# TuringLang/AdvancedVI.jl

Hardware: AMD Instinct MI355X
Metric: ELBO-grad-estimates/sec (higher is better)
Workload: dtype f32

## Files before the change

advancedvi.jl_amd/csrc/device_common.h:

```cpp
#pragma once
#include "mivi_internal.h"
#include "philox.h"
#include <type_traits>

namespace mivi {

template <typename T>
__device__ __forceinline__ T wave_sum(T v) {
#pragma unroll
  for (int o = 32; o > 0; o >>= 1) v += __shfl_xor(v, o, 64);
  return v;
}

__device__ __forceinline__ float wave_sum_f32(float v) {
  v += __builtin_bit_cast(float, __builtin_amdgcn_update_dpp(0, __builtin_bit_cast(int, v), 0xB1, 0xF, 0xF, true));
  v += __builtin_bit_cast(float, __builtin_amdgcn_update_dpp(0, __builtin_bit_cast(int, v), 0x4E, 0xF, 0xF, true));
  v += __builtin_bit_cast(float, __builtin_amdgcn_update_dpp(0, __builtin_bit_cast(int, v), 0x141, 0xF, 0xF, true));
  v += __builtin_bit_cast(float, __builtin_amdgcn_update_dpp(0, __builtin_bit_cast(int, v), 0x140, 0xF, 0xF, true));
  const int iv = __builtin_bit_cast(int, v);
  return __builtin_bit_cast(float, __builtin_amdgcn_readlane(iv, 0)) + __builtin_bit_cast(float, __builtin_amdgcn_readlane(iv, 16)) +
         __builtin_bit_cast(float, __builtin_amdgcn_readlane(iv, 32)) + __builtin_bit_cast(float, __builtin_amdgcn_readlane(iv, 48));
}
__device__ __forceinline__ double wave_sum_fast(float v) { return (double)wave_sum_f32(v); }
__device__ __forceinline__ double wave_sum_fast(double v) { return wave_sum(v); }

template <typename T, int NT>
__device__ __forceinline__ T block_sum(T v, T *red) {
  const int lane = threadIdx.x & 63, w = threadIdx.x >> 6;
  v = wave_sum(v);
  __syncthreads();
  if (lane == 0) red[w] = v;
  __syncthreads();
  T s = red[0];
#pragma unroll
  for (int i = 1; i < NT / 64; ++i) s += red[i];
  return s;
}

__device__ __forceinline__ void lds_barrier();
template <typename T, int NT>
__device__ __forceinline__ T block_sum_nodrain(T v, T *red) {
  const int lane = threadIdx.x & 63, w = threadIdx.x >> 6;
  v = wave_sum(v);
  lds_barrier();
  if (lane == 0) red[w] = v;
  lds_barrier();
  T s = red[0];
#pragma unroll
  for (int i = 1; i < NT / 64; ++i) s += red[i];
  return s;
}

template <int NT>
__device__ __forceinline__ double block_sum_nodrain_f32(float v, double *red) {
  const int lane = threadIdx.x & 63, w = threadIdx.x >> 6;
  const double sv = (double)wave_sum_f32(v);
  lds_barrier();
  if (lane == 0) red[w] = sv;
  lds_barrier();
  double s = red[0];
#pragma unroll
  for (int i = 1; i < NT / 64; ++i) s += red[i];
  return s;
}

template <typename T, int NT, int N>
__device__ __forceinline__ void block_sum_n(T (&v)[N], T *red) {
  const int lane = threadIdx.x & 63, w = threadIdx.x >> 6;
#pragma unroll
  for (int k = 0; k < N; ++k) v[k] = wave_sum(v[k]);
  __syncthreads();
  if (lane == 0) {
#pragma unroll
    for (int k = 0; k < N; ++k) red[k * (NT / 64) + w] = v[k];
  }
  __syncthreads();
#pragma unroll
  for (int k = 0; k < N; ++k) {
    T s = red[k * (NT / 64)];
#pragma unroll
    for (int i = 1; i < NT / 64; ++i) s += red[k * (NT / 64) + i];
    v[k] = s;
  }
}

template <int B, int E, typename F>
__device__ __forceinline__ void static_for(F &&f) {
  if constexpr (B < E) {
    f(std::integral_constant<int, B>{});
    static_for<B + 1, E>(f);
  }
}

template <typename V16>
__device__ __forceinline__ void store16_wt(void *p, const V16 &v) {
  static_assert(sizeof(V16) == 16, "16-byte vector");
  typedef unsigned u32x4_t __attribute__((ext_vector_type(4)));
  const u32x4_t r = __builtin_bit_cast(u32x4_t, v);
  asm volatile("global_store_dwordx4 %0, %1, off sc1\n\ts_nop 1" ::"v"(p), "v"(r) : "memory");
}

__device__ __forceinline__ void store4_wt(float *p, float v) {
  asm volatile("global_store_dword %0, %1, off sc1" ::"v"(p), "v"(v) : "memory");
}

#ifdef MIVI_DEV
#define MIVI_STAMP_K(dbgp, kind, slot) do { if ((dbgp) && threadIdx.x == 0 && blockIdx.x < 4096) (dbgp)[((size_t)(kind) * 4096 + blockIdx.x) * 8 + (slot)] = wall_clock64(); } while (0)
#define MIVI_KNOCKED(args, bits) ((args).knock & (bits))
#define MIVI_DEV_ONLY(...) __VA_ARGS__
#else
#define MIVI_STAMP_K(dbgp, kind, slot) do { } while (0)
#define MIVI_KNOCKED(args, bits) false
#define MIVI_DEV_ONLY(...)
#endif
#define MIVI_STAMP(dbgp, slot) MIVI_STAMP_K(dbgp, 0, slot)

__device__ __forceinline__ void lds_barrier() { asm volatile("s_waitcnt lgkmcnt(0)\n\ts_barrier" ::: "memory"); }

__device__ __forceinline__ uint64_t rng_index(const RngArgs &r) {
  return r.idx_base + (r.idx_ptr ? *r.idx_ptr : 0ull);
}

__device__ __forceinline__ double direct_entropy_coeff(int ent_kind) {
  switch (ent_kind) {
    case MIVI_ENT_CLOSED_FORM: return 1.0;
    case MIVI_ENT_CLOSED_FORM_ZERO_GRAD: return 0.0;
    case MIVI_ENT_MONTE_CARLO: return 1.0;
    case MIVI_ENT_STL: return 0.0;
    default: return -1.0;
  }
}

__device__ __forceinline__ bool ent_is_stl(int k) { return k == MIVI_ENT_STL || k == MIVI_ENT_STL_ZERO_GRAD; }
__device__ __forceinline__ bool ent_is_closed(int k) {
  return k == MIVI_ENT_CLOSED_FORM || k == MIVI_ENT_CLOSED_FORM_ZERO_GRAD;
}

template <typename T>
__device__ __forceinline__ T mf_grad_entry(double row_sum, double invM, bool scale_row, double direct, double sigma) {
#pragma clang fp contract(off)
  const double m = -row_sum * invM;
  const double e = direct / sigma;
  return (T)(scale_row ? m - e : m);
}

template <bool ATOMIC>
__device__ __forceinline__ double ld_f64(const double *p) {
  if (ATOMIC) return __hip_atomic_load(p, __ATOMIC_RELAXED, __HIP_MEMORY_SCOPE_AGENT);
  return *p;
}

template <typename T, int NT, bool ATOMIC = false>
__device__ __forceinline__ void funnel_finish(int d, const FunnelFin &f, const OutArgs &out, double &s_ell, double &sW, double &sWe) {
  const int tid = threadIdx.x;
  const T *params = (const T *)f.params;
  const double mu0 = f.row0 ? (double)__hip_atomic_load((const T *)f.row0, __ATOMIC_RELAXED, __HIP_MEMORY_SCOPE_AGENT) : (double)params[0];
  const double sg0 = f.row0 ? (double)__hip_atomic_load((const T *)f.row0 + 1, __ATOMIC_RELAXED, __HIP_MEMORY_SCOPE_AGENT) : (double)params[d];
  const uint64_t idx = rng_index(f.rng);
  const bool stl = ent_is_stl(out.ent_kind);
  const double n = (double)(d - 1), sv2 = f.sigma_v * f.sigma_v;
  for (int m = tid; m < f.M; m += NT) {
#pragma clang fp contract(off)
    T e[4];
    eps_block<T>(f.rng.seed, idx, (uint64_t)(f.rng.m_offset + m) * (uint64_t)f.d4, e);
    const double e0 = (double)e[0];
    const double e1 = (double)fma((T)sg0, e[0], (T)mu0);
    s_ell += (-e1 - e1 * e1 / (2.0 * sv2)) + (-n * e1) + e1;
    const double w = (-1.0 - e1 / sv2) + (-n) + 1.0 + (stl ? e0 / sg0 : 0.0);
    sW += w;
    sWe += w * e0;
  }
  if (f.wait_word) {
    for (int i = tid; i < f.wait_n; i += NT) {
      int budget = f.wait_budget;
      while ((int)(__hip_atomic_load(f.wait_word + i, __ATOMIC_RELAXED, __HIP_MEMORY_SCOPE_AGENT) - f.wait_val) < 0) {
        if (--budget <= 0) { if (out.status) atomicOr(out.status, 8); break; }
        __builtin_amdgcn_s_sleep(1);
      }
    }
    __syncthreads();
    asm volatile("" ::: "memory");
    if (f.mirror) {
      constexpr int UN = 8;
      for (int base = 0; base < f.mirror_n; base += UN * NT) {
        double v[UN];
#pragma unroll
        for (int u = 0; u < UN; ++u) {
          const int i = base + u * NT + tid;
          v[u] = i < f.mirror_n ? f.mirror_src[i] : 0.0;
        }
#pragma unroll
        for (int u = 0; u < UN; ++u) {
          const int i = base + u * NT + tid;
          if (i < f.mirror_n) f.mirror[i] = v[u];
        }
      }
      __syncthreads();
    }
  }
  for (int i = tid; i < f.n_part; i += NT) {
    sW += ld_f64<ATOMIC>(f.ab + i);
    sWe += ld_f64<ATOMIC>(f.ab + f.n_part + i);
  }
}

struct PartialDst {
  float *flat;
  const P2PDirectTab *tab;
  long long n, off;
  float inv_n;
};
__device__ __forceinline__ PartialDst partial_dst(const OutArgs &out) {
  PartialDst pd;
  pd.flat = (float *)out.partials;
  pd.tab = (const P2PDirectTab *)out.p2p_direct;
  pd.n = 1; pd.off = 0; pd.inv_n = 1.f;
  if (pd.tab) {
    const unsigned epoch = __hip_atomic_load(pd.tab->ctr, __ATOMIC_RELAXED, __HIP_MEMORY_SCOPE_AGENT) + 1u + (unsigned)out.p2p_gi;
    pd.n = pd.tab->n;
    pd.off = ((long long)((int)(epoch & 1u) * pd.tab->GV + out.p2p_v) * pd.tab->R + pd.tab->rank) * pd.n;
    pd.inv_n = 1.f / (float)pd.n;
  }
  return pd;
}
__device__ __forceinline__ void partial_store(const PartialDst &pd, long long idx, float v) {
  if (!pd.tab) { pd.flat[idx] = v; return; }
  int s = (int)((float)idx * pd.inv_n);
  if (s > pd.tab->R - 1) s = pd.tab->R - 1;
  while ((long long)s * pd.n > idx) --s;
  while ((long long)(s + 1) * pd.n <= idx) ++s;
  float *dst = (float *)pd.tab->stage[s] + pd.off + (idx - (long long)s * pd.n);
  __hip_atomic_store(dst, v, __ATOMIC_RELAXED, __HIP_MEMORY_SCOPE_SYSTEM);
}

template <typename T, int NT, bool ATOMIC, bool FUNNEL = false, typename DiagFn>
__device__ void finalize_value_block(int d, const ValueIn &vin, const OutArgs &out, int64_t plen, DiagFn scale_diag,
                                     double *red) {
  const int tid = threadIdx.x;
  double s_ell = 0.0, s_he = 0.0, s_ld = 0.0, bad = 0.0, sW = 0.0, sWe = 0.0;
  const bool funnel = FUNNEL && vin.fn.ab;
  if (funnel) funnel_finish<T, NT, ATOMIC>(d, vin.fn, out, s_ell, sW, sWe);
  for (int i = tid; i < vin.n_ell_part; i += NT) s_ell += ld_f64<ATOMIC>(vin.ell_part + i);
  for (int i = tid; i < vin.n_ell_part2; i += NT) s_ell += ld_f64<ATOMIC>(vin.ell_part2 + i);
  for (int i = tid; i < vin.n_ell; i += NT) s_ell += (double)((const T *)vin.ell)[i];
  for (int i = tid; i < vin.n_he_part; i += NT) s_he += ld_f64<ATOMIC>(vin.he_part + i);
  if (!out.partials_mode) {
    if (vin.ld_part) {
      for (int i = tid; i < vin.n_ld_part; i += NT) {
        s_ld += ld_f64<ATOMIC>(vin.ld_part + i);
        bad += ld_f64<ATOMIC>(vin.ld_part + vin.n_ld_part + i);
      }
    } else {
      for (int i = tid; i < d; i += NT) {
        const double c = (double)scale_diag(i);
// ... 57 lines not shown
```

advancedvi.jl_amd/csrc/fr_planes.h:

```cpp
#pragma once
#include "device_common.h"

namespace mivi {

typedef float f32x16 __attribute__((ext_vector_type(16)));
typedef float f32x4 __attribute__((ext_vector_type(4)));
typedef _Float16 f16x8 __attribute__((ext_vector_type(8)));
typedef _Float16 f16x2 __attribute__((ext_vector_type(2)));
typedef unsigned u32x4v __attribute__((ext_vector_type(4)));

constexpr int kFrag = 512;
constexpr int kSplitProducts = 3;
constexpr float kEpsScale = 2048.f;
constexpr float kEpsInv = 1.f / 2048.f;

#define FB_GLDS16(gptr, lptr, off)                                                                         \
  __builtin_amdgcn_global_load_lds((const __attribute__((address_space(1))) void *)(gptr),                 \
                                   (__attribute__((address_space(3))) void *)(lptr), 16, off, 0)

template <int N>
__device__ __forceinline__ void fb_wait_vm() {
  __builtin_amdgcn_s_waitcnt((N & 15) | (7 << 4) | (15 << 8) | ((N >> 4) << 14));
  asm volatile("" ::: "memory");
}
__device__ __forceinline__ void fb_barrier() {
  __builtin_amdgcn_s_waitcnt(0xc07f);
  asm volatile("s_barrier" ::: "memory");
}

__device__ __forceinline__ void fb_scale_of(float amax, float &s, float &inv) {
  unsigned eb = (__builtin_bit_cast(unsigned, amax) >> 23) & 0xffu;
  eb = eb < 25u ? 25u : (eb > 254u ? 254u : eb);
  s = __builtin_bit_cast(float, (267u - eb) << 23);
  inv = __builtin_bit_cast(float, (eb - 13u) << 23);
}

__device__ __forceinline__ void fb_split2(const float *x, u32x4v &uh, u32x4v &ul) {
#pragma unroll
  for (int p = 0; p < 4; ++p) {
    const float a = x[2 * p], b = x[2 * p + 1];
    const _Float16 ah = (_Float16)a, bh = (_Float16)b;
    const float ra = a - (float)ah, rb = b - (float)bh;
    const f16x2 hh = {ah, bh}, ll = {(_Float16)ra, (_Float16)rb};
    uh[p] = __builtin_bit_cast(unsigned, hh);
    ul[p] = __builtin_bit_cast(unsigned, ll);
  }
}
__device__ __forceinline__ float fb_unsplit2(const u32x4v &uh, const u32x4v &ul, int e) {
  const unsigned wh = uh[e >> 1], wl = ul[e >> 1];
  const f16x2 hh = __builtin_bit_cast(f16x2, wh), ll = __builtin_bit_cast(f16x2, wl);
  return (float)hh[e & 1] + (float)ll[e & 1];
}
__device__ __forceinline__ float fb_unsplit2_word(unsigned wh, unsigned wl, int odd) {
  const f16x2 hh = __builtin_bit_cast(f16x2, wh), ll = __builtin_bit_cast(f16x2, wl);
  return (float)hh[odd] + (float)ll[odd];
}
__device__ __forceinline__ void fb_store_frag(unsigned *dst, const float *x) {
  u32x4v uh, ul;
  fb_split2(x, uh, ul);
  store16_wt(dst, uh);
  store16_wt(dst + 256, ul);
}

constexpr int kStageW = 16 * 256;

template <int WJ>
struct FbFrags {
  u32x4v A[2][2], B[WJ][2];
};
__device__ __forceinline__ f32x16 fb_mma(const u32x4v &a, const u32x4v &b, const f32x16 &c) {
  return __builtin_amdgcn_mfma_f32_32x32x16_f16(__builtin_bit_cast(f16x8, a), __builtin_bit_cast(f16x8, b), c, 0, 0, 0);
}
template <int WJ>
__device__ __forceinline__ void fb_group(const FbFrags<WJ> &F, f32x16 (&acc)[2][WJ]) {
  constexpr int PA[3] = {1, 0, 0}, PB[3] = {0, 1, 0};
#pragma unroll
  for (int p = 0; p < 3; ++p)
#pragma unroll
    for (int i = 0; i < 2; ++i)
#pragma unroll
      for (int j = 0; j < WJ; ++j) acc[i][j] = fb_mma(F.A[i][PA[p]], F.B[j][PB[p]], acc[i][j]);
}

template <int OFF>
__device__ __forceinline__ void fb_group_read_asm(f32x16 &acc0, f32x16 &acc1, const FbFrags<1> &Fc, FbFrags<1> &Fn, unsigned ab, unsigned bb) {
  static_assert(OFF >= 0 && OFF + 3072 < 65536, "ds_read_b128 offset field");
  asm volatile(
      "v_mfma_f32_32x32x16_f16 %[c0], %[a0l], %[bh], %[c0]\n\t"
      "ds_read_b128 %[n0h], %[ab] offset:%[o0]\n\t"
      "ds_read_b128 %[n0l], %[ab] offset:%[o1]\n\t"
      "v_mfma_f32_32x32x16_f16 %[c1], %[a1l], %[bh], %[c1]\n\t"
      "ds_read_b128 %[n1h], %[ab] offset:%[o2]\n\t"
      "ds_read_b128 %[n1l], %[ab] offset:%[o3]\n\t"
      "v_mfma_f32_32x32x16_f16 %[c0], %[a0h], %[bl], %[c0]\n\t"
      "ds_read_b128 %[nbh], %[bb] offset:%[o0]\n\t"
      "v_mfma_f32_32x32x16_f16 %[c1], %[a1h], %[bl], %[c1]\n\t"
      "ds_read_b128 %[nbl], %[bb] offset:%[o1]\n\t"
      "v_mfma_f32_32x32x16_f16 %[c0], %[a0h], %[bh], %[c0]\n\t"
      "v_mfma_f32_32x32x16_f16 %[c1], %[a1h], %[bh], %[c1]\n\t"
      "s_waitcnt lgkmcnt(0)"
      : [c0] "+v"(acc0), [c1] "+v"(acc1), [n0h] "=&v"(Fn.A[0][0]), [n0l] "=&v"(Fn.A[0][1]), [n1h] "=&v"(Fn.A[1][0]), [n1l] "=&v"(Fn.A[1][1]),
        [nbh] "=&v"(Fn.B[0][0]), [nbl] "=&v"(Fn.B[0][1])
      : [a0h] "v"(Fc.A[0][0]), [a0l] "v"(Fc.A[0][1]), [a1h] "v"(Fc.A[1][0]), [a1l] "v"(Fc.A[1][1]), [bh] "v"(Fc.B[0][0]), [bl] "v"(Fc.B[0][1]),
        [ab] "v"(ab), [bb] "v"(bb), [o0] "n"(OFF), [o1] "n"(OFF + 1024), [o2] "n"(OFF + 2048), [o3] "n"(OFF + 3072)
      : "memory");
}

template <int WJ>
__device__ __forceinline__ void fb_read_frags(const unsigned *lds, int slot, int wm, int wn, int lane, FbFrags<WJ> &F) {
  const unsigned *cur = lds + slot * kStageW + 4 * lane;
#pragma unroll
  for (int i = 0; i < 2; ++i)
#pragma unroll
    for (int p = 0; p < 2; ++p) F.A[i][p] = *(const u32x4v *)(cur + ((2 * wm + i) * 2 + p) * 256);
#pragma unroll
  for (int j = 0; j < WJ; ++j)
#pragma unroll
    for (int p = 0; p < 2; ++p) F.B[j][p] = *(const u32x4v *)(cur + (8 + (WJ * wn + j) * 2 + p) * 256);
}

}
```

advancedvi.jl_amd/csrc/kernels_fullrank_batch.hip:

```cpp
#include <algorithm>
#include <cstdlib>
#include <type_traits>
#include <cstdio>
#include <vector>

#include "device_common.h"
#include "fr_elem.h"
#include "fr_planes.h"

#ifndef FB_VK
#define FB_VK 0
#endif
#ifndef FB_WJ
#define FB_WJ 1
#endif

namespace mivi {

struct FbArgs {
  int d, M, L;
  int dT, MT;
  const float *params;
  const float *t_mean, *t_istd;
  unsigned *CA;
  float *cscale;
  unsigned *epsP;
  unsigned *WV;
  float *winv;
  const float *t_prec;
  int dP;
  unsigned *PA;
  float *pscale;
  unsigned *RP;
  float *rinv;
  const float *Tinv;
  unsigned *TA;
  float *tscale;
  long long plane_stride;
  double *ell_part;
  long long ell_stride;
  double *he_part;
  long long he_stride;
  double *ld_part;
  const int4 *work;
  int n_work;
  float *grads;
  long long grad_stride;
  float *values;
  long long value_stride;
  float *grad_last, *value_last;
  int lane_last;
  int write_upper;
  int ent_kind, M_total;
  int *status;
  double ell_const;
  RngArgs rng;
  int n_riders;
  int obj;
  float *parts;
  long long part_stride;
  int knock;
  long long *dbg;
};
#ifdef MIVI_DEV
#define FB_STAMP(a, slot) do { if ((a).dbg && threadIdx.x == 0) (a).dbg[(size_t)blockIdx.x * 8 + (slot)] = (long long)wall_clock64(); } while (0)
#define FB_NOTE(a, slot, v) do { if ((a).dbg && threadIdx.x == 0) (a).dbg[(size_t)blockIdx.x * 8 + (slot)] = (long long)(v); } while (0)
#define FB_KNOCKED(a, b) ((a).knock & (b))
#else
#define FB_KNOCKED(a, b) false
#define FB_STAMP(a, slot) do { } while (0)
#define FB_NOTE(a, slot, v) do { } while (0)
#endif

template <class Ld4, class Ld>
__device__ __forceinline__ void fb_rowblock_planes(int d, int rb, int kg_lo, int kg_hi, int sub, int nsub, Ld4 ld4, Ld ld, unsigned *planes, float *scale, float *red) {
  const int tid = threadIdx.x, r4 = tid & 7, part = tid >> 3, ng = d >> 4;
  f32x4 m = {0.f, 0.f, 0.f, 0.f};
  {
    int k = 16 * kg_lo + part;
    for (; k + 448 <= 16 * kg_hi + 15; k += 512) {
      f32x4 v[8];
#pragma unroll
      for (int u = 0; u < 8; ++u) v[u] = ld4(k + 64 * u, 32 * rb + 4 * r4);
#pragma unroll
      for (int u = 0; u < 8; ++u)
#pragma unroll
        for (int c = 0; c < 4; ++c) m[c] = fmaxf(m[c], fabsf(v[u][c]));
    }
    for (; k <= 16 * kg_hi + 15; k += 64) {
      const f32x4 v = ld4(k, 32 * rb + 4 * r4);
#pragma unroll
      for (int c = 0; c < 4; ++c) m[c] = fmaxf(m[c], fabsf(v[c]));
    }
  }
#pragma unroll
  for (int c = 0; c < 4; ++c) {
    m[c] = fmaxf(m[c], __shfl_xor(m[c], 8, 64));
    m[c] = fmaxf(m[c], __shfl_xor(m[c], 16, 64));
    m[c] = fmaxf(m[c], __shfl_xor(m[c], 32, 64));
  }
  if ((tid & 63) < 8) *(f32x4 *)(red + (tid >> 6) * 32 + 4 * r4) = m;
  lds_barrier();
  if (tid < 32) {
    float mm = red[tid];
#pragma unroll
    for (int p = 1; p < 8; ++p) mm = fmaxf(mm, red[p * 32 + tid]);
    float s, inv;
    fb_scale_of(mm, s, inv);
    red[512 + tid] = s;
    if (sub == 0) {
      scale[32 * rb + tid] = s;
      scale[d + 32 * rb + tid] = inv;
    }
  }
  lds_barrier();
  const int w = tid >> 6, lane = tid & 63, l31 = lane & 31, h = lane >> 5;
  const float s = red[512 + l31];
  for (int kg = kg_lo + w + 8 * sub; kg <= kg_hi; kg += 8 * nsub) {
    float x[8];
#pragma unroll
    for (int e = 0; e < 8; ++e) x[e] = ld(16 * kg + 8 * (e >> 2) + 4 * h + (e & 3), 32 * rb + l31) * s;
    fb_store_frag(planes + ((size_t)rb * ng + kg) * kFrag + 4 * lane, x);
  }
}
__device__ __forceinline__ void fb_cplanes_block(const FbArgs &a, int rb, int sub, int nsub, float *red) {
  const int d = a.d, ng = d >> 4, dT = a.dT;
  const float *C = a.params + dT;
  const int hi = 2 * rb + 3 < ng - 1 ? 2 * rb + 3 : ng - 1;
  if (dT == d) {
    fb_rowblock_planes(d, rb, 0, hi, sub, nsub,
                       [C, d](int k, int row) { f32x4 v = *(const f32x4 *)(C + (size_t)k * d + row);
#pragma unroll
                                                for (int c = 0; c < 4; ++c) v[c] = k > row + c ? 0.f : v[c];
                                                return v; },
                       [C, d](int k, int row) { const float v = C[(size_t)k * d + row]; return k > row ? 0.f : v; }, a.CA, a.cscale, red);
    return;
  }
  fb_rowblock_planes(d, rb, 0, hi, sub, nsub,
                     [C, dT](int k, int row) { const bool in = row < dT && k < dT;
                                               f32x4 v = *(const f32x4 *)(C + (size_t)(in ? k : 0) * dT + (in ? row : 0));
#pragma unroll
                                               for (int c = 0; c < 4; ++c) v[c] = (!in || k > row + c) ? 0.f : v[c];
                                               return v; },
                     [C, dT](int k, int row) { if (row >= dT || k > row) return 0.f; return C[(size_t)k * dT + row]; }, a.CA, a.cscale, red);
}
__global__ __launch_bounds__(512) void k_fb_pplanes(FbArgs a) {
  __shared__ float red[16 * 32 + 32];
  const float *P = a.t_prec;
  const int dP = a.dP;
  fb_rowblock_planes(a.d, (int)blockIdx.x, 0, (a.d >> 4) - 1, (int)blockIdx.y, (int)gridDim.y,
                     [P, dP](int k, int row) { return *(const f32x4 *)(P + (size_t)k * dP + row); },
                     [P, dP](int k, int row) { return P[(size_t)k * dP + row]; }, a.PA, a.pscale, red);
}
__global__ __launch_bounds__(512) void k_fb_tplanes(FbArgs a) {
  __shared__ float red[16 * 32 + 32];
  const float *T = a.Tinv;
  const int d = a.d, rb = (int)blockIdx.x;
  fb_rowblock_planes(d, rb, 2 * (rb & ~3), (d >> 4) - 1, (int)blockIdx.y, (int)gridDim.y,
                     [T, d](int k, int row) { f32x4 v = *(const f32x4 *)(T + (size_t)k * d + row);
#pragma unroll
                                              for (int c = 0; c < 4; ++c) v[c] = k >= row + c ? v[c] : 0.f;
                                              return v; },
                     [T, d](int k, int row) { const float v = T[(size_t)k * d + row]; return k >= row ? v : 0.f; }, a.TA, a.tscale, red);
}

__global__ __launch_bounds__(512) void k_fb_eps(FbArgs a) {
  __shared__ double red[8];
  __shared__ float E[32 * 65];
  const int tid = threadIdx.x, eb = blockIdx.x, d = a.d;
  if ((int)blockIdx.y < a.n_riders) {
    const int r = (int)blockIdx.y * (int)gridDim.x + eb;
    if (r < 4 * (d >> 5)) fb_cplanes_block(a, (d >> 5) - 1 - (r >> 2), r & 3, 4, E);
    return;
  }
  const int l = (int)blockIdx.y - a.n_riders;
  const uint64_t idx = rng_index(a.rng) + (a.obj ? 0ull : (uint64_t)l);
  const int moff = a.rng.m_offset + (a.obj ? l * a.MT : 0);
  unsigned *epsP = a.epsP + (size_t)l * a.plane_stride;
  const int nrb6 = d >> 6;
  const int R64 = eb % nrb6, c32 = eb / nrb6;
  const int q = tid & 15, c = tid >> 4;
  const int ri = R64 * 64 + 4 * q, rm = c32 * 32 + c;
  float e[4];
  eps_block<float>(a.rng.seed, idx, (uint64_t)(moff + rm) * (uint64_t)(a.dT >> 2) + (uint64_t)(ri >> 2), e);
  if (!(ri < a.dT && rm < a.MT)) { e[0] = 0.f; e[1] = 0.f; e[2] = 0.f; e[3] = 0.f; }
#pragma unroll
  for (int r = 0; r < 4; ++r) E[c * 65 + 4 * q + r] = e[r] * kEpsScale;
  const float he = 0.5f * (e[0] * e[0] + e[1] * e[1] + e[2] * e[2] + e[3] * e[3]);
  const double sh = block_sum_nodrain_f32<512>(he, red);
  if (tid == 0) a.he_part[(size_t)l * a.he_stride + eb] = sh;
  if (tid >= 256) return;
  const int lane = tid & 63, l31 = lane & 31, h = lane >> 5, f = tid >> 6;
  float x[8];
#pragma unroll
  for (int s = 0; s < 8; ++s) x[s] = E[l31 * 65 + 16 * f + 8 * (s >> 2) + 4 * h + (s & 3)];
  fb_store_frag(epsP + ((size_t)c32 * (d >> 4) + 4 * R64 + f) * kFrag + 4 * lane, x);
}

constexpr int kImgW = 32 * 36;
template <int WJ>
__device__ __forceinline__ void fb_sched_interleave() {
  constexpr int NM = 6 * WJ, ND = 4 + 2 * WJ, NV = 2 * WJ;
  static_for<0, NM>([&](auto K) {
    constexpr int k = decltype(K)::value;
    constexpr int nrd = (k + 1) * ND / NM - k * ND / NM;
    __builtin_amdgcn_sched_group_barrier(0x008, 1, 0);
    if constexpr (nrd > 0) __builtin_amdgcn_sched_group_barrier(0x100, nrd, 0);
    if constexpr (k < NV) __builtin_amdgcn_sched_group_barrier(0x020, 1, 0);
  });
}
using FbI0 = std::integral_constant<int, 0>;
using FbI1 = std::integral_constant<int, 1>;
using FbI2 = std::integral_constant<int, 2>;
using FbI3 = std::integral_constant<int, 3>;
using FbT = std::true_type;
using FbN = std::false_type;

template <int MASK>
__device__ __forceinline__ float fb_lane_max(float v) {
#pragma unroll
  for (int o = 1; o < 64; o <<= 1)
    if (MASK & o) v = fmaxf(v, __shfl_xor(v, o, 64));
  return v;
}

enum { FB_DIAG = 0, FB_DENSE_R = 1, FB_DENSE_G = 2, FB_STL_U = 3 };
template <int WJ, int MODE, int NRP>
__global__ __launch_bounds__(512 / WJ, (MODE == 2 && NRP == 4 && WJ == 1) ? 4 : 2 / WJ) void k_fb_prod(FbArgs a) {
  constexpr bool kDG = MODE == FB_DENSE_G, kSU = MODE == FB_STL_U, kDR = MODE == FB_DENSE_R;
  constexpr int LDC = 36, NF = WJ, kPW = 2 * WJ;
  constexpr int NW = 8 / WJ, NWN = 4 / WJ;
  constexpr int kBody = (NRP * kStageW > 16 * kImgW) ? NRP * kStageW : 16 * kImgW;
  constexpr bool kTabInBody = kDG && NRP * kStageW + 2048 <= kBody;
  constexpr int kTab = kDG ? (kTabInBody ? 128 : 2048 + 128) : 0;
  __shared__ __attribute__((aligned(16))) unsigned lds[kBody + 4 * 128 + NW * 64 + kTab];
  float *vec = reinterpret_cast<float *>(lds + kBody);
  float *red = vec + 4 * 128;
  float *rsv = red + NW * 64;
  float *tab = kTabInBody ? reinterpret_cast<float *>(lds + NRP * kStageW) : rsv + 128;
  const int tid = threadIdx.x, lane = tid & 63, l31 = lane & 31, h = lane >> 5;
  const int w = __builtin_amdgcn_readfirstlane(tid >> 6);
  const int wm = w / NWN, wn = w % NWN;
  const __attribute__((address_space(4))) int *wp = (const __attribute__((address_space(4))) int *)a.work + 4 * blockIdx.x;
  const int ln = wp[0], rc = wp[1], flags = wp[2];
  const int rb = rc & 0xffff, cb = rc >> 16;
  const int d = a.d, ng = d >> 4;
  const int row0 = rb * 128, col0 = cb * 128;
  const int R0 = row0 >> 5;
  const int g0 = kSU ? 2 * R0 : 0;
  const int G = kDG ? ng : (kSU ? ng - g0 : 2 * (R0 + 4));
  const unsigned *sp[NF];
  int gmax[NF];
#pragma unroll
  for (int f = 0; f < NF; ++f) {
    const int fs = NF * w + f, fr = fs & 3;
    if (fs < 4) {
      sp[f] = (kDG ? a.PA : (kSU ? a.TA : a.CA)) + ((size_t)(R0 + fr) * ng + g0) * kFrag + 4 * lane;
      gmax[f] = (!kDG && !kSU && 2 * (R0 + fr) + 3 < G - 1) ? 2 * (R0 + fr) + 3 : G - 1;
    } else {
      sp[f] = (kDG ? a.RP : a.epsP) + (size_t)ln * a.plane_stride + ((size_t)((col0 >> 5) + fr) * ng + g0) * kFrag + 4 * lane;
      gmax[f] = G - 1;
    }
  }
  int gd = 0;
  constexpr int kMaxNB = 16;
  float tv[4] = {0.f, 0.f, 0.f, 0.f}, tri[kDG ? kMaxNB : 1], trs = 0.f;
  auto load_tables = [&]() {
    if (tid < 128) {
      if constexpr (!kDG && !kSU) {
        const bool in = row0 + tid < a.dT;
        tv[0] = in ? a.params[row0 + tid] : 0.f;
        tv[1] = in ? a.t_mean[row0 + tid] : 0.f;
        if (MODE == FB_DIAG) tv[2] = in ? a.t_istd[row0 + tid] : 0.f;
      }
      const float *sc = kDG ? a.pscale : (kSU ? a.tscale : a.cscale);
      tv[3] = sc[d + row0 + tid];
      if constexpr (kDG) {
        const float *ri = a.rinv + (size_t)ln * (size_t)(d >> 7) * a.M + col0 + tid;
        const int NB = d >> 7;
#pragma unroll
        for (int b = 0; b < kMaxNB; ++b) tri[b] = ri[(size_t)(b < NB ? b : NB - 1) * a.M];
        trs = ri[(size_t)rb * a.M];
      }
    }
    asm volatile("" ::: "memory");
  };
  auto stage_tables = [&]() {
    if (tid < 128) {
      if constexpr (!kDG && !kSU) {
        vec[tid] = tv[0];
        vec[128 + tid] = tv[1];
        if (MODE == FB_DIAG) vec[256 + tid] = tv[2];
      }
      vec[384 + tid] = tv[3] * ((kDG) ? 1.f : kEpsInv);
      if constexpr (kDG) {
        const int NB = d >> 7;
        float u = tri[0], grow = 1.f;
#pragma unroll
        for (int b = 1; b < kMaxNB; ++b) {
          if (b < NB) {
            float ratio = u / tri[b];
            if (!(ratio <= 1099511627776.f)) ratio = 1099511627776.f;
            if (ratio > 1.f && grow * ratio > 1.2089258e24f) ratio = fmaxf(1.2089258e24f / grow, 1.f);
            if (ratio > 1.f) grow *= ratio;
            tab[(b - 1) * 128 + tid] = ratio;
            u = u / ratio;
          }
        }
        tab[(NB - 1) * 128 + tid] = u;
        rsv[tid] = trs;
      }
    }
  };
  auto issue = [&](int slot) {
#pragma unroll
    for (int f = 0; f < NF; ++f) {
      unsigned *dst = lds + slot * kStageW + (NF * w + f) * 512;
      FB_GLDS16(sp[f], dst, 0);
      FB_GLDS16(sp[f], dst, 1024);
      sp[f] += gd < gmax[f] ? kFrag : 0;
    }
    ++gd;
  };
  f32x16 acc[2][WJ];
#pragma unroll
  for (int i = 0; i < 2; ++i)
#pragma unroll
    for (int j = 0; j < WJ; ++j)
#pragma unroll
      for (int r = 0; r < 16; ++r) acc[i][j][r] = 0.f;
  const int r32[2] = {R0 + 2 * wm, R0 + 2 * wm + 1};
  const int Gw = (kDG || kSU) ? G : 2 * r32[1] + 2;
  auto after_group = [&](auto S, int g) {
    if constexpr (kDG && (decltype(S)::value & 3) == 3) {
      if (((g + 1) & 7) == 0) {
#pragma unroll
        for (int j = 0; j < WJ; ++j) {
          const float f = tab[((g >> 3) << 7) + 32 * (WJ * wn + j) + l31];
#pragma unroll
          for (int i = 0; i < 2; ++i) {
#pragma unroll
            for (int r = 0; r < 16; ++r) acc[i][j][r] *= f;
          }
        }
        asm volatile("" ::: "memory");
      }
    }
  };
  auto compute = [&](auto S, int g, const FbFrags<WJ> &F) {
// ... 569 lines not shown
constexpr int kOwnCuTilesPerCU10 = 17;

void fb_upload(DevBuf &b, const void *src, size_t bytes) {
  if (b.bytes < bytes || !b.p) {
    if (b.p) (void)hipFree(b.p);
    (void)hipMalloc(&b.p, bytes);
    b.bytes = bytes;
  }
  (void)hipMemcpy(b.p, src, bytes, hipMemcpyHostToDevice);
}
}

static int fb_pad(int x) { return (x + 127) / 128 * 128; }
bool fb_shape_ok(const mivi_ctx *c, int M) {
  static const bool off = getenv("MIVI_BATCH_GEN3") && atoi(getenv("MIVI_BATCH_GEN3")) == 0;
  return !off && c->cfg.family == MIVI_FULLRANK && c->cfg.dtype == MIVI_F32 && c->cfg.d % 32 == 0 && M % 32 == 0 && c->cfg.d >= kBM &&
         c->cfg.d <= 2048 && M >= 128 && M <= 2048;
}
bool fb_whole_tiles(const mivi_ctx *c, int M) { return c->cfg.d % kBM == 0 && M % kBN == 0; }
size_t fb_plane_words(const mivi_ctx *c, int M) { return (size_t)fb_pad(c->cfg.d) * fb_pad(M) / 512 * kFrag; }
size_t fb_cplane_words(const mivi_ctx *c) { return (size_t)(fb_pad(c->cfg.d) / 32) * (fb_pad(c->cfg.d) / 16) * kFrag; }
size_t fb_part_len(const mivi_ctx *c) {
  const size_t d = (size_t)c->cfg.d, T = d / 128;
  return (d + T * (T + 1) / 2 * 16384 + 2 + 3) / 4 * 4;
}

const FbTab *fb_prepare(mivi_ctx *c, int M, int L) {
  FbTables &ft = c->fb;
  for (FbTab &t : ft.tab)
    if (t.L == L && t.M == M && t.prod.p && t.vjp.p) return &t;
  FbTab &t = ft.tab[ft.next_tab];
  ft.next_tab = (ft.next_tab + 1) & 3;
  invalidate_graph(c);
  (void)hipStreamSynchronize(c->stream);
  t.L = t.M = 0;
  const int d = fb_pad(c->cfg.d), nrb = d / kBM, ncb = fb_pad(M) / kBN;
  std::vector<std::vector<int4>> lists(8);
  int panel = 0;
  for (int l = 0; l < L; ++l)
    for (int cb = 0; cb < ncb; ++cb, ++panel)
      for (int rb = nrb - 1; rb >= 0; --rb) lists[panel % 8].push_back(make_int4(l, rb | (cb << 16), (l == 0 && cb == 0) ? 1 : 0, 0));
  while (true) {
    int a = 0, b = 0;
    for (int x = 1; x < 8; ++x) {
      if (lists[x].size() > lists[a].size()) a = x;
      if (lists[x].size() < lists[b].size()) b = x;
    }
    if (lists[a].size() <= lists[b].size() + 1) break;
    lists[b].push_back(lists[a].back());
    lists[a].pop_back();
  }
  for (auto &li : lists) std::stable_sort(li.begin(), li.end(), [](const int4 &p, const int4 &q) { return (p.y & 0xffff) > (q.y & 0xffff); });
  std::vector<int4> prod;
  size_t mx = 0;
  for (auto &li : lists) mx = std::max(mx, li.size());
  for (size_t i = 0; i < mx; ++i)
    for (int x = 0; x < 8; ++x)
      if (i < lists[x].size()) prod.push_back(lists[x][i]);
  std::vector<int4> flat;
  for (int l = 0; l < L; ++l)
    for (int rb = 0; rb < nrb; ++rb)
      for (int cb = 0; cb <= rb; ++cb) flat.push_back(make_int4(l, rb | (cb << 16), 0, 0));
  std::vector<int4> vjp;
  {
    const size_t n = flat.size();
    size_t pos = 0;
    std::vector<std::vector<int4>> lx(8);
    for (int x = 0; x < 8; ++x) {
      const size_t e = (n * (x + 1)) / 8;
      for (; pos < e; ++pos) lx[x].push_back(flat[pos]);
    }
    size_t m2 = 0;
    for (auto &li : lx) m2 = std::max(m2, li.size());
    for (size_t i = 0; i < m2; ++i)
      for (int x = 0; x < 8; ++x)
        if (i < lx[x].size()) vjp.push_back(lx[x][i]);
  }
  std::vector<int4> prod2;
  const size_t panel_bytes = (size_t)kBM * d * 4;
  constexpr int NG = 4, NC = 8 / NG;
  if (nrb % NG == 0 && (size_t)(nrb / NG) * panel_bytes <= (1u << 20)) {
    std::vector<std::vector<int4>> lp(8);
    int pn = 0;
    for (int l = 0; l < L; ++l)
      for (int cb = 0; cb < ncb; ++cb, ++pn)
        for (int rg = 0; rg < NG; ++rg)
          for (int r = 0; r < nrb / NG; ++r) lp[rg + NG * (pn % NC)].push_back(make_int4(l, (rg * (nrb / NG) + r) | (cb << 16), 0, 0));
    size_t m3 = 0;
    for (auto &li : lp) m3 = std::max(m3, li.size());
    for (size_t i = 0; i < m3; ++i)
      for (int x = 0; x < 8; ++x)
        if (i < lp[x].size()) prod2.push_back(lp[x][i]);
  } else {
    for (int l = 0; l < L; ++l)
      for (int cb = 0; cb < ncb; ++cb)
        for (int rb = 0; rb < nrb; ++rb) prod2.push_back(make_int4(l, rb | (cb << 16), 0, 0));
  }
  std::vector<int4> prod3;
  for (auto &li : lists) std::stable_sort(li.begin(), li.end(), [](const int4 &p, const int4 &q) { return (p.y & 0xffff) < (q.y & 0xffff); });
  for (size_t i = 0; i < mx; ++i)
    for (int x = 0; x < 8; ++x)
      if (i < lists[x].size()) prod3.push_back(lists[x][i]);
  fb_upload(t.prod, prod.data(), prod.size() * sizeof(int4));
  fb_upload(t.vjp, vjp.data(), vjp.size() * sizeof(int4));
  fb_upload(t.prod2, prod2.data(), prod2.size() * sizeof(int4));
  fb_upload(t.prod3, prod3.data(), prod3.size() * sizeof(int4));
  if (!t.prod.p || !t.vjp.p || !t.prod2.p || !t.prod3.p) return nullptr;
  t.n_prod2 = (int)prod2.size();
  t.n_prod = (int)prod.size();
  t.n_vjp = (int)vjp.size();
  t.L = L;
  t.M = M;
  return &t;
}

static FbArgs fb_args(mivi_ctx *c, const void *params, int M_true) {
  FbTables &t = c->fb;
  const int d = fb_pad(c->cfg.d), M = fb_pad(M_true);
  FbArgs a{};
  a.d = d; a.M = M;
  a.dT = c->cfg.d; a.MT = M_true;
  a.params = (const float *)params;
  a.t_mean = (const float *)c->t_mean.p;
  a.t_istd = (const float *)c->t_istd.p;
  a.CA = (unsigned *)t.CA.p;
  a.cscale = (float *)t.cscale.p;
  a.pscale = (float *)t.pscale.p;
  a.tscale = (float *)t.tscale.p;
  a.winv = (float *)t.winv.p;
  a.rinv = (float *)t.rinv.p;
  a.epsP = (unsigned *)t.epsP.p;
  a.WV = (unsigned *)t.WV.p;
  a.t_prec = (const float *)c->t_prec.p; a.dP = c->dP;
  a.PA = (unsigned *)t.PA.p;
  a.RP = (unsigned *)t.RP.p;
  a.Tinv = (const float *)t.Tinv.p;
  a.TA = (unsigned *)t.TA.p;
  a.plane_stride = (long long)fb_plane_words(c, M);
  a.ell_part = (double *)t.ell.p; a.ell_stride = (long long)(d / 32) * (M / 32);
  a.he_part = (double *)t.he.p; a.he_stride = (long long)(d / 64) * (M / 32);
  a.ld_part = (double *)t.ld.p;
  a.ent_kind = c->cfg.entropy; a.M_total = c->M_total;
  a.status = (int *)c->status.p;
  a.ell_const = c->t_const;
  return a;
}

void fb_launch_eps(mivi_ctx *c, const FbStep &s, bool with_cplanes, hipStream_t stream) {
  const int d = fb_pad(c->cfg.d), M = fb_pad(s.M), L = s.L;
  FbArgs a = fb_args(c, s.params, s.M);
  a.L = L;
  a.rng = s.rng;
  a.obj = s.obj;
  const int gx = (d / 64) * (M / 32);
  a.n_riders = with_cplanes ? (4 * (d / 32) + gx - 1) / gx : 0;
  hipLaunchKernelGGL(k_fb_eps, dim3(gx, L + a.n_riders), dim3(512), 0, stream, a);
}
void fb_launch_pplanes(mivi_ctx *c, hipStream_t stream) {
  FbArgs a = fb_args(c, nullptr, c->cfg.n_mc);
  hipLaunchKernelGGL(k_fb_pplanes, dim3(c->cfg.d / 32, 4), dim3(512), 0, stream, a);
}
void fb_launch_tplanes(mivi_ctx *c, hipStream_t stream) {
  FbArgs a = fb_args(c, nullptr, c->cfg.n_mc);
  hipLaunchKernelGGL(k_fb_tplanes, dim3(c->cfg.d / 32, 4), dim3(512), 0, stream, a);
}
void fb_launch_compute(mivi_ctx *c, const FbStep &s, hipStream_t stream, int which) {
  const FbTab &tb = *s.tab;
  FbArgs a = fb_args(c, s.params, s.M);
  a.L = s.L;
  a.grads = (float *)s.grads; a.grad_stride = s.grad_stride;
  a.values = (float *)s.values; a.value_stride = s.value_stride;
  a.grad_last = (float *)s.grad_last; a.value_last = (float *)s.value_last; a.lane_last = s.lane_last;
  a.write_upper = s.write_upper;
  a.parts = (float *)s.parts; a.part_stride = s.part_stride;
  if (s.obj) { a.ent_kind = s.ent_kind; a.M_total = s.M; }
#ifdef MIVI_DEV
  static long long *dbg_buf = nullptr;
  static const bool dbg_on = getenv("MIVI_FB_DBG") != nullptr;
  if (dbg_on && !dbg_buf) (void)hipMalloc(&dbg_buf, 2 * 8192 * 8 * sizeof(long long));
  auto dump = [&](const char *name, int n) {
    if (!dbg_on) return;
    (void)hipStreamSynchronize(stream);
    std::vector<long long> h((size_t)n * 8);
    (void)hipMemcpy(h.data(), dbg_buf, h.size() * 8, hipMemcpyDeviceToHost);
    long long t0 = h[0], t3 = 0;
    for (int i = 0; i < n; ++i) { t0 = std::min(t0, h[(size_t)i * 8]); t3 = std::max(t3, h[(size_t)i * 8 + 3]); }
    double pro = 0, loop = 0, epi = 0, pg = 0; long long gs = 0;
    for (int i = 0; i < n; ++i) { const long long *r = &h[(size_t)i * 8]; pro += r[1] - r[0]; loop += r[2] - r[1]; epi += r[3] - r[2]; gs += r[4]; }
    pg = loop / (double)gs;
    fprintf(stderr, "[fbdbg] %s: %d workgroups, span %.2f us | mean prologue %.2f us, main loop %.2f us (%.3f us per group), epilogue %.2f us | last start %.2f us\n", name, n, (t3 - t0) * 0.01, pro / n * 0.01, loop / n * 0.01, pg * 0.01, epi / n * 0.01, 0.0);
    std::vector<long long> st; for (int i = 0; i < n; ++i) st.push_back(h[(size_t)i * 8] - t0);
    std::sort(st.begin(), st.end());
    fprintf(stderr, "[fbdbg]   starts (us): p25 %.2f p50 %.2f p75 %.2f p90 %.2f max %.2f\n", st[n / 4] * 0.01, st[n / 2] * 0.01, st[3 * n / 4] * 0.01, st[9 * n / 10] * 0.01, st[n - 1] * 0.01);
  };
  a.dbg = dbg_on ? dbg_buf : nullptr;
  a.knock = getenv("MIVI_FB_KNOCK") ? atoi(getenv("MIVI_FB_KNOCK")) : 0;
#endif
  a.work = (const int4 *)tb.prod.p; a.n_work = tb.n_prod;
  const int n_cu = c->n_cu > 0 ? c->n_cu : 256;
  auto own_cu_for = [&](int n, bool equal_tiles) {
#ifdef MIVI_DEV
    static const int force_ring = getenv("MIVI_FB_RING") ? atoi(getenv("MIVI_FB_RING")) : 0;
    if (force_ring == 4) return false;
    if (force_ring == 8) return true;
#endif
    const int gmax = fb_pad(c->cfg.d) / 16;
    const int thr10 = gmax <= 32 ? 10 : (gmax <= 64 ? 10 + (gmax - 32) * 7 / 32 : kOwnCuTilesPerCU10 + (gmax - 64 < 64 ? gmax - 64 : 64) * 5 / 64);
    return !equal_tiles && n > n_cu && 10 * (long long)n <= (long long)thr10 * n_cu;
  };
  auto prod = [&](auto MODE, int n) {
    constexpr int md = decltype(MODE)::value;
    if (own_cu_for(n, md == FB_DENSE_G)) hipLaunchKernelGGL((k_fb_prod<kWJ, md, 8>), dim3(n), dim3(512 / kWJ), 0, stream, a);
    else hipLaunchKernelGGL((k_fb_prod<kWJ, md, 4>), dim3(n), dim3(512 / kWJ), 0, stream, a);
  };
  if (s.dense) {
    if (which & 1) prod(std::integral_constant<int, FB_DENSE_R>{}, tb.n_prod);
    a.work = (const int4 *)tb.prod2.p; a.n_work = tb.n_prod2;
    if (which & 4) prod(std::integral_constant<int, FB_DENSE_G>{}, tb.n_prod2);
  } else if (which & 1) {
    prod(std::integral_constant<int, FB_DIAG>{}, tb.n_prod);
#ifdef MIVI_DEV
    dump("k_fb_prod<DIAG>", tb.n_prod);
#endif
  }
  if (s.stl && (which & 8)) {
    a.work = (const int4 *)tb.prod3.p; a.n_work = tb.n_prod;
    prod(std::integral_constant<int, FB_STL_U>{}, tb.n_prod);
  }
  a.work = (const int4 *)tb.vjp.p; a.n_work = tb.n_vjp;
  if (s.values_only) {
    if (which & 2) hipLaunchKernelGGL((k_fb_vjp<kWJ, 3, 256, 6>), dim3(s.L), dim3(512 / kWJ), 0, stream, a);
    return;
  }
  if (which & 2) {
    if (s.parts) {
      if (a.M <= 256) hipLaunchKernelGGL((k_fb_vjp<kWJ, 3, 256, 6, true>), dim3(tb.n_vjp + s.L), dim3(512 / kWJ), 0, stream, a);
      else hipLaunchKernelGGL((k_fb_vjp<kWJ, 3, 2048, 4, true>), dim3(tb.n_vjp + s.L), dim3(512 / kWJ), 0, stream, a);
    }
    else if (a.M <= 256) hipLaunchKernelGGL((k_fb_vjp<kWJ, 3, 256, 6>), dim3(tb.n_vjp + s.L), dim3(512 / kWJ), 0, stream, a);
    else hipLaunchKernelGGL((k_fb_vjp<kWJ, 3, 2048, 4>), dim3(tb.n_vjp + s.L), dim3(512 / kWJ), 0, stream, a);
#ifdef MIVI_DEV
    dump("k_fb_vjp", tb.n_vjp);
#endif
  }
}

void fb_launch_finalize_parts(mivi_ctx *c, const FbStep &s, hipStream_t stream) {
  FbArgs a = fb_args(c, s.params, s.M);
  a.L = s.L;
  a.grads = (float *)s.grads; a.grad_stride = s.grad_stride;
  a.values = (float *)s.values; a.value_stride = s.value_stride;
  a.grad_last = (float *)s.grad_last; a.value_last = (float *)s.value_last; a.lane_last = s.lane_last;
  a.write_upper = s.write_upper;
  a.parts = (float *)s.parts; a.part_stride = s.part_stride;
  hipLaunchKernelGGL(k_fb_finalize_parts, dim3(c->cfg.d + 1, s.L), dim3(256), 0, stream, a);
}

}
```

advancedvi.jl_amd/csrc/philox.h:

```cpp
#pragma once
#include <stdint.h>

#if defined(__HIPCC__)
#define MIVI_HD __host__ __device__ __forceinline__
#else
#define MIVI_HD inline
#endif

namespace mivi {

struct u32x4 {
  uint32_t x, y, z, w;
};

MIVI_HD uint32_t mulhi32(uint32_t a, uint32_t b) {
#if defined(__HIP_DEVICE_COMPILE__)
  return __umulhi(a, b);
#else
  return (uint32_t)(((uint64_t)a * (uint64_t)b) >> 32);
#endif
}

MIVI_HD u32x4 philox4x32_10(u32x4 c, uint32_t k0, uint32_t k1) {
  const uint32_t M0 = 0xD2511F53u, M1 = 0xCD9E8D57u, W0 = 0x9E3779B9u, W1 = 0xBB67AE85u;
#pragma unroll
  for (int r = 0; r < 10; ++r) {
    const uint64_t p0 = (uint64_t)M0 * (uint64_t)c.x, p1 = (uint64_t)M1 * (uint64_t)c.z;
    const uint32_t hi0 = (uint32_t)(p0 >> 32), lo0 = (uint32_t)p0;
    const uint32_t hi1 = (uint32_t)(p1 >> 32), lo1 = (uint32_t)p1;
    u32x4 n;
#if defined(__HIP_DEVICE_COMPILE__) && defined(__gfx950__)
    n.x = __builtin_amdgcn_bitop3_b32(hi1, c.y, k0, 0x96);
    n.z = __builtin_amdgcn_bitop3_b32(hi0, c.w, k1, 0x96);
#else
    n.x = hi1 ^ c.y ^ k0;
    n.z = hi0 ^ c.w ^ k1;
#endif
    n.y = lo1;
    n.w = lo0;
    c = n;
    k0 += W0;
    k1 += W1;
  }
  return c;
}

MIVI_HD u32x4 eps_block_bits(uint64_t seed, uint64_t idx, uint64_t q) {
  u32x4 c;
  c.x = (uint32_t)q;
  c.y = (uint32_t)(q >> 32);
  c.z = (uint32_t)idx;
  c.w = (uint32_t)(idx >> 32);
  return philox4x32_10(c, (uint32_t)seed, (uint32_t)(seed >> 32));
}

template <typename T>
struct BoxMuller;

template <>
struct BoxMuller<float> {
  static MIVI_HD void pair(uint32_t wa, uint32_t wb, float &n0, float &n1) {
    const float ua = ((float)(wa >> 9) + 0.5f) * 1.1920928955078125e-07f;
    const float ub = ((float)(wb >> 9) + 0.5f) * 1.1920928955078125e-07f;
#if defined(__HIP_DEVICE_COMPILE__) && !defined(MIVI_LIBM_BOXMULLER)
    const float r = __builtin_amdgcn_sqrtf(-1.38629436111989f * __builtin_amdgcn_logf(ua));
    const float x4 = 4.0f * ub;
    const float qf = __builtin_rintf(x4);
    const float th = (x4 - qf) * 1.57079632679489662f;
    const float t2 = th * th;
    const float ps = __builtin_fmaf(t2, __builtin_fmaf(t2, -1.9515295891e-4f, 8.3321608736e-3f), -1.6666654611e-1f);
    const float sp = __builtin_fmaf(th * t2, ps, th);
    const float pc = __builtin_fmaf(t2, __builtin_fmaf(t2, 2.443315711809948e-5f, -1.388731625493765e-3f), 4.166664568298827e-2f);
    const float cp = __builtin_fmaf(t2 * t2, pc, __builtin_fmaf(-0.5f, t2, 1.0f));
    const unsigned qi = (unsigned)(int)qf;
    const bool swap = (qi & 1u) != 0u;
    const unsigned ss = (qi & 2u) << 30, cs = ((qi + 1u) & 2u) << 30;
    const float s = __builtin_bit_cast(float, __builtin_bit_cast(unsigned, swap ? cp : sp) ^ ss);
    const float c = __builtin_bit_cast(float, __builtin_bit_cast(unsigned, swap ? sp : cp) ^ cs);
#elif defined(__HIP_DEVICE_COMPILE__)
    const float r = sqrtf(-2.0f * logf(ua));
    float s, c;
    sincospif(2.0f * ub, &s, &c);
#else
    const float r = (float)__builtin_sqrt(-2.0 * __builtin_log((double)ua));
    const double ang = 6.283185307179586476925286766559 * (double)ub;
    const float s = (float)__builtin_sin(ang), c = (float)__builtin_cos(ang);
#endif
    n0 = r * c;
    n1 = r * s;
#if defined(__HIP_DEVICE_COMPILE__)
    asm volatile("" : "+v"(n0), "+v"(n1));
#endif
  }
};

template <>
struct BoxMuller<double> {
  static MIVI_HD void pair(uint32_t wa, uint32_t wb, double &n0, double &n1) {
    const double ua = ((double)wa + 0.5) * 2.3283064365386962890625e-10;
    const double ub = ((double)wb + 0.5) * 2.3283064365386962890625e-10;
#if defined(__HIP_DEVICE_COMPILE__)
    const double r = sqrt(-2.0 * log(ua));
    double s, c;
    sincospi(2.0 * ub, &s, &c);
#else
    const double r = __builtin_sqrt(-2.0 * __builtin_log(ua));
    const double ang = 6.283185307179586476925286766559 * ub;
    const double s = __builtin_sin(ang), c = __builtin_cos(ang);
#endif
    n0 = r * c;
    n1 = r * s;
  }
};

template <typename T>
MIVI_HD void eps_block(uint64_t seed, uint64_t idx, uint64_t q, T out[4]) {
  const u32x4 b = eps_block_bits(seed, idx, q);
  BoxMuller<T>::pair(b.x, b.y, out[0], out[1]);
  BoxMuller<T>::pair(b.z, b.w, out[2], out[3]);
}

}
```

Before: 353,700.

## Make eps kernel persistent with double-buffered LDS and packed Box-Muller

New measurement: 349,700 (median of 2 runs). About the same (-1.1%).

```diff
diff --git a/advancedvi.jl_amd/csrc/device_common.h b/advancedvi.jl_amd/csrc/device_common.h
--- a/advancedvi.jl_amd/csrc/device_common.h
+++ b/advancedvi.jl_amd/csrc/device_common.h
@@ -100,6 +100,12 @@
   asm volatile("global_store_dwordx4 %0, %1, off sc1\n\ts_nop 1" ::"v"(p), "v"(r) : "memory");
 }
 
+template <typename V8>
+__device__ __forceinline__ void store8_wt(void *p, const V8 &v) {
+  static_assert(sizeof(V8) == 8, "8-byte vector");
+  typedef unsigned u32x2_t __attribute__((ext_vector_type(2)));
+  asm volatile("global_store_dwordx2 %0, %1, off sc1" ::"v"(p), "v"(__builtin_bit_cast(u32x2_t, v)) : "memory");
+}
 __device__ __forceinline__ void store4_wt(float *p, float v) {
   asm volatile("global_store_dword %0, %1, off sc1" ::"v"(p), "v"(v) : "memory");
 }
diff --git a/advancedvi.jl_amd/csrc/fr_planes.h b/advancedvi.jl_amd/csrc/fr_planes.h
--- a/advancedvi.jl_amd/csrc/fr_planes.h
+++ b/advancedvi.jl_amd/csrc/fr_planes.h
@@ -8,6 +8,7 @@
 typedef _Float16 f16x8 __attribute__((ext_vector_type(8)));
 typedef _Float16 f16x2 __attribute__((ext_vector_type(2)));
 typedef unsigned u32x4v __attribute__((ext_vector_type(4)));
+typedef unsigned u32x2v __attribute__((ext_vector_type(2)));
 
 constexpr int kFrag = 512;
 constexpr int kSplitProducts = 3;
@@ -35,15 +36,20 @@
   inv = __builtin_bit_cast(float, (eb - 13u) << 23);
 }
 
+__device__ __forceinline__ void fb_split_word(float a, float b, unsigned &wh, unsigned &wl) {
+  const _Float16 ah = (_Float16)a, bh = (_Float16)b;
+  const float ra = a - (float)ah, rb = b - (float)bh;
+  const f16x2 hh = {ah, bh}, ll = {(_Float16)ra, (_Float16)rb};
+  wh = __builtin_bit_cast(unsigned, hh);
+  wl = __builtin_bit_cast(unsigned, ll);
+}
 __device__ __forceinline__ void fb_split2(const float *x, u32x4v &uh, u32x4v &ul) {
 #pragma unroll
   for (int p = 0; p < 4; ++p) {
-    const float a = x[2 * p], b = x[2 * p + 1];
-    const _Float16 ah = (_Float16)a, bh = (_Float16)b;
-    const float ra = a - (float)ah, rb = b - (float)bh;
-    const f16x2 hh = {ah, bh}, ll = {(_Float16)ra, (_Float16)rb};
-    uh[p] = __builtin_bit_cast(unsigned, hh);
-    ul[p] = __builtin_bit_cast(unsigned, ll);
+    unsigned wh, wl;
+    fb_split_word(x[2 * p], x[2 * p + 1], wh, wl);
+    uh[p] = wh;
+    ul[p] = wl;
   }
 }
 __device__ __forceinline__ float fb_unsplit2(const u32x4v &uh, const u32x4v &ul, int e) {
@@ -60,6 +66,18 @@
   fb_split2(x, uh, ul);
   store16_wt(dst, uh);
   store16_wt(dst + 256, ul);
+}
+__device__ __forceinline__ void fb_store_frag_half(unsigned *dst, const float *x) {
+  u32x2v uh, ul;
+#pragma unroll
+  for (int p = 0; p < 2; ++p) {
+    unsigned wh, wl;
+    fb_split_word(x[2 * p], x[2 * p + 1], wh, wl);
+    uh[p] = wh;
+    ul[p] = wl;
+  }
+  store8_wt(dst, uh);
+  store8_wt(dst + 256, ul);
 }
 
 constexpr int kStageW = 16 * 256;
diff --git a/advancedvi.jl_amd/csrc/kernels_fullrank_batch.hip b/advancedvi.jl_amd/csrc/kernels_fullrank_batch.hip
--- a/advancedvi.jl_amd/csrc/kernels_fullrank_batch.hip
+++ b/advancedvi.jl_amd/csrc/kernels_fullrank_batch.hip
@@ -166,35 +166,45 @@
 
 __global__ __launch_bounds__(512) void k_fb_eps(FbArgs a) {
   __shared__ double red[8];
-  __shared__ float E[32 * 65];
-  const int tid = threadIdx.x, eb = blockIdx.x, d = a.d;
-  if ((int)blockIdx.y < a.n_riders) {
-    const int r = (int)blockIdx.y * (int)gridDim.x + eb;
-    if (r < 4 * (d >> 5)) fb_cplanes_block(a, (d >> 5) - 1 - (r >> 2), r & 3, 4, E);
+  __shared__ float E[2][32 * 65];
+  const int tid = threadIdx.x, d = a.d;
+  if ((int)blockIdx.x < a.n_riders) {
+    const int r = (int)blockIdx.x;
+    fb_cplanes_block(a, (d >> 5) - 1 - (r >> 2), r & 3, 4, E[0]);
     return;
   }
-  const int l = (int)blockIdx.y - a.n_riders;
-  const uint64_t idx = rng_index(a.rng) + (a.obj ? 0ull : (uint64_t)l);
-  const int moff = a.rng.m_offset + (a.obj ? l * a.MT : 0);
-  unsigned *epsP = a.epsP + (size_t)l * a.plane_stride;
-  const int nrb6 = d >> 6;
-  const int R64 = eb % nrb6, c32 = eb / nrb6;
+  const int nrb6 = d >> 6, gx = nrb6 * (a.M >> 5), n_items = a.L * gx, n_draw = (int)gridDim.x - a.n_riders;
   const int q = tid & 15, c = tid >> 4;
-  const int ri = R64 * 64 + 4 * q, rm = c32 * 32 + c;
-  float e[4];
-  eps_block<float>(a.rng.seed, idx, (uint64_t)(moff + rm) * (uint64_t)(a.dT >> 2) + (uint64_t)(ri >> 2), e);
-  if (!(ri < a.dT && rm < a.MT)) { e[0] = 0.f; e[1] = 0.f; e[2] = 0.f; e[3] = 0.f; }
-#pragma unroll
-  for (int r = 0; r < 4; ++r) E[c * 65 + 4 * q + r] = e[r] * kEpsScale;
-  const float he = 0.5f * (e[0] * e[0] + e[1] * e[1] + e[2] * e[2] + e[3] * e[3]);
-  const double sh = block_sum_nodrain_f32<512>(he, red);
-  if (tid == 0) a.he_part[(size_t)l * a.he_stride + eb] = sh;
-  if (tid >= 256) return;
-  const int lane = tid & 63, l31 = lane & 31, h = lane >> 5, f = tid >> 6;
-  float x[8];
-#pragma unroll
-  for (int s = 0; s < 8; ++s) x[s] = E[l31 * 65 + 16 * f + 8 * (s >> 2) + 4 * h + (s & 3)];
-  fb_store_frag(epsP + ((size_t)c32 * (d >> 4) + 4 * R64 + f) * kFrag + 4 * lane, x);
+  const int f = tid >> 7, lane = (tid >> 1) & 63, s4 = tid & 1, l31 = lane & 31, h = lane >> 5;
+  const uint64_t idx0 = rng_index(a.rng);
+  int buf = 0;
+  for (int item = (int)blockIdx.x - a.n_riders; item < n_items; item += n_draw, buf ^= 1) {
+    const int l = item / gx, eb = item - l * gx;
+    const uint64_t idx = idx0 + (a.obj ? 0ull : (uint64_t)l);
+    const int moff = a.rng.m_offset + (a.obj ? l * a.MT : 0);
+    const int R64 = eb % nrb6, c32 = eb / nrb6;
+    const int ri = R64 * 64 + 4 * q, rm = c32 * 32 + c;
+    float e[4];
+    BoxMuller<float>::quad(eps_block_bits(a.rng.seed, idx, (uint64_t)(moff + rm) * (uint64_t)(a.dT >> 2) + (uint64_t)(ri >> 2)), e);
+    if (!(ri < a.dT && rm < a.MT)) { e[0] = 0.f; e[1] = 0.f; e[2] = 0.f; e[3] = 0.f; }
+    float *Eb = E[buf];
+#pragma unroll
+    for (int r = 0; r < 4; ++r) Eb[c * 65 + 4 * q + r] = e[r] * kEpsScale;
+    const double hw = (double)wave_sum_f32(0.5f * (e[0] * e[0] + e[1] * e[1] + e[2] * e[2] + e[3] * e[3]));
+    lds_barrier();
+    if ((tid & 63) == 0) red[tid >> 6] = hw;
+    lds_barrier();
+    if (tid == 0) {
+      double sh = red[0];
+#pragma unroll
+      for (int i = 1; i < 8; ++i) sh += red[i];
+      a.he_part[(size_t)l * a.he_stride + eb] = sh;
+    }
+    float x[4];
+#pragma unroll
+    for (int s = 0; s < 4; ++s) x[s] = Eb[l31 * 65 + 16 * f + 8 * s4 + 4 * h + s];
+    fb_store_frag_half(a.epsP + (size_t)l * a.plane_stride + ((size_t)c32 * (d >> 4) + 4 * R64 + f) * kFrag + 4 * lane + 2 * s4, x);
+  }
 }
 
 constexpr int kImgW = 32 * 36;
@@ -1070,9 +1080,15 @@
   a.L = L;
   a.rng = s.rng;
   a.obj = s.obj;
-  const int gx = (d / 64) * (M / 32);
-  a.n_riders = with_cplanes ? (4 * (d / 32) + gx - 1) / gx : 0;
-  hipLaunchKernelGGL(k_fb_eps, dim3(gx, L + a.n_riders), dim3(512), 0, stream, a);
+  a.n_riders = with_cplanes ? 4 * (d / 32) : 0;
+  static const int per_cu = [] {
+    int n = 0;
+    if (hipOccupancyMaxActiveBlocksPerMultiprocessor(&n, k_fb_eps, 512, 0) != hipSuccess || n < 1) { (void)hipGetLastError(); n = 3; }
+    return n;
+  }();
+  const int items = (d / 64) * (M / 32) * L, round = per_cu * (c->n_cu > 0 ? c->n_cu : 256);
+  const int avail = round > a.n_riders ? round - a.n_riders : round, k = (items + avail - 1) / avail;
+  hipLaunchKernelGGL(k_fb_eps, dim3(a.n_riders + (items + k - 1) / k), dim3(512), 0, stream, a);
 }
 void fb_launch_pplanes(mivi_ctx *c, hipStream_t stream) {
   FbArgs a = fb_args(c, nullptr, c->cfg.n_mc);
diff --git a/advancedvi.jl_amd/csrc/philox.h b/advancedvi.jl_amd/csrc/philox.h
--- a/advancedvi.jl_amd/csrc/philox.h
+++ b/advancedvi.jl_amd/csrc/philox.h
@@ -92,6 +92,45 @@
     asm volatile("" : "+v"(n0), "+v"(n1));
 #endif
   }
+#if defined(__HIPCC__)
+  static __device__ __forceinline__ void quad(const u32x4 &w, float out[4]) {
+#if defined(__HIP_DEVICE_COMPILE__) && !defined(MIVI_LIBM_BOXMULLER)
+    typedef float f2 __attribute__((ext_vector_type(2)));
+    const f2 one_a = {__builtin_bit_cast(float, __builtin_amdgcn_alignbit(0x7fu, w.x, 9u)), __builtin_bit_cast(float, __builtin_amdgcn_alignbit(0x7fu, w.z, 9u))};
+    const f2 one_b = {__builtin_bit_cast(float, __builtin_amdgcn_alignbit(0x7fu, w.y, 9u)), __builtin_bit_cast(float, __builtin_amdgcn_alignbit(0x7fu, w.w, 9u))};
+    const f2 ua = one_a - 0x1.fffffep-1f, ub = one_b - 0x1.fffffep-1f;
+    const f2 lg = {__builtin_amdgcn_logf(ua.x), __builtin_amdgcn_logf(ua.y)};
+    const f2 rr = -1.38629436111989f * lg;
+    const f2 r = {__builtin_amdgcn_sqrtf(rr.x), __builtin_amdgcn_sqrtf(rr.y)};
+    const f2 x4 = 4.0f * ub;
+    const f2 qf = {__builtin_rintf(x4.x), __builtin_rintf(x4.y)};
+    const f2 th = (x4 - qf) * 1.57079632679489662f;
+    const f2 t2 = th * th;
+    const f2 ps = __builtin_elementwise_fma(t2, __builtin_elementwise_fma(t2, (f2)(-1.9515295891e-4f), (f2)(8.3321608736e-3f)), (f2)(-1.6666654611e-1f));
+    const f2 sp = __builtin_elementwise_fma(th * t2, ps, th);
+    const f2 pc = __builtin_elementwise_fma(t2, __builtin_elementwise_fma(t2, (f2)(2.443315711809948e-5f), (f2)(-1.388731625493765e-3f)), (f2)(4.166664568298827e-2f));
+    const f2 cp = __builtin_elementwise_fma(t2 * t2, pc, __builtin_elementwise_fma((f2)(-0.5f), t2, (f2)(1.0f)));
+    f2 s, c;
+#pragma unroll
+    for (int k = 0; k < 2; ++k) {
+      const unsigned qi = (unsigned)(int)qf[k];
+      const bool swap = (qi & 1u) != 0u;
+      const unsigned ss = (qi & 2u) << 30, cs = ((qi + 1u) & 2u) << 30;
+      s[k] = __builtin_bit_cast(float, __builtin_bit_cast(unsigned, swap ? cp[k] : sp[k]) ^ ss);
+      c[k] = __builtin_bit_cast(float, __builtin_bit_cast(unsigned, swap ? sp[k] : cp[k]) ^ cs);
+    }
+    f2 n0 = r * c, n1 = r * s;
+    asm volatile("" : "+v"(n0), "+v"(n1));
+    out[0] = n0.x;
+    out[1] = n1.x;
+    out[2] = n0.y;
+    out[3] = n1.y;
+#else
+    pair(w.x, w.y, out[0], out[1]);
+    pair(w.z, w.w, out[2], out[3]);
+#endif
+  }
+#endif
 };
 
 template <>
```
